# Bob-cheng/DepthModelHardening

Measured on AMD Instinct MI355X. Metric: adv-train images/sec @1024x320, 10-step PGD, bs32, higher is better.
Workload: dtype f32; 1 GPU; Monodepth2 ResNet18 1024x320, 10-step PGD-L_inf attack on 12 scenes, train batch 32/GPU, stereo photometric+SSIM+smoothness loss (md2), Adam; config_index=2, global_batch=32, per_gpu_batch=32, parallelism=dp1, attack_overlap=False, attack_scenes=12, graph_attack=False

## Files before the change

depthmodelhardening_amd/_native.py:

```python
import ctypes as C
import os

import torch

MAX_SCALES = 4
MAX_FRAMES = 4
VARIANT_MD2, VARIANT_DH = 0, 1
NOISE_NONE, NOISE_TENSOR, NOISE_PHILOX = 0, 1, 2
PASTE_COMPOSITE, PASTE_WARP_ONLY = 0, 1
FIN_LOSS, FIN_LOSS_S, FIN_REPROJ_S, FIN_COUNT_S, FIN_SMOOTH_S, FIN_HINT_S, FIN_HINTCOUNT_S, FIN_SIZE = 0, 1, 5, 9, 13, 20, 24, 28

LIB_PATH = os.environ.get("DMH_HIP_LIB") or os.path.join(os.path.dirname(os.path.abspath(__file__)), "lib",
                                                        "libdmh_hip.so")

_fp = C.c_void_p


class PhotoArgs(C.Structure):
    _fields_ = [("target", _fp), ("source", _fp * MAX_FRAMES), ("T", _fp * MAX_FRAMES), ("K", _fp), ("inv_K", _fp),
                ("disp", _fp * MAX_SCALES), ("Hs", C.c_int * MAX_SCALES), ("Ws", C.c_int * MAX_SCALES),
                ("B", C.c_int), ("H", C.c_int), ("W", C.c_int), ("num_frames", C.c_int), ("num_scales", C.c_int),
                ("min_depth", C.c_float), ("max_depth", C.c_float), ("variant", C.c_int), ("automask", C.c_int),
                ("no_ssim", C.c_int), ("noise_mode", C.c_int), ("noise", _fp * MAX_SCALES),
                ("seed", C.c_uint64), ("offset", C.c_uint64), ("depth_hint", _fp), ("depth_hint_mask", _fp)]
# ... 91 lines not shown
    "dmh_conv7x7s2_bwd_data_win": (C.c_int, [_fp] * 4 + [C.c_int] * 9 + [_fp, _fp]),
    "dmh_roi_cost_partials_size": (C.c_int64, [C.c_int, C.c_int, C.c_int]),
    "dmh_roi_cost_fwd": (C.c_int, [_fp, _fp, _fp] + [C.c_int] * 5 + [_fp] * 4),
    "dmh_roi_cost_bwd": (C.c_int, [_fp, _fp, _fp] + [C.c_int] * 5 + [_fp] * 3),
    "dmh_roi_cost_fwd_scaled": (C.c_int, [_fp, _fp, _fp] + [C.c_int] * 5 + [C.c_float] + [_fp] * 4),
    "dmh_roi_cost_bwd_scaled": (C.c_int, [_fp, _fp, _fp] + [C.c_int] * 5 + [C.c_float] + [_fp] * 3),
    "dmh_bn_act_fwd": (C.c_int, [_fp] * 4 + [C.c_int] * 4 + [_fp, _fp]),
    "dmh_bn_act_bwd": (C.c_int, [_fp] * 3 + [C.c_int] * 4 + [_fp, _fp, _fp]),
    "dmh_bn_stats_partials_size": (C.c_int64, [C.c_int, C.c_int, C.c_int]),
    "dmh_bn_train_stats": (C.c_int, [_fp, C.c_int, C.c_int, C.c_int, _fp, _fp, C.c_float, C.c_float] + [_fp] * 8),
    "dmh_bn_train_stats_tracked": (C.c_int, [_fp, C.c_int, C.c_int, C.c_int, _fp, _fp, C.c_float, C.c_float] + [_fp] * 9),
    "dmh_channel_sum_partials_size": (C.c_int64, [C.c_int, C.c_int, C.c_int]),
    "dmh_channel_sum": (C.c_int, [_fp, C.c_int, C.c_int, C.c_int, _fp, _fp, C.c_void_p]),
    "dmh_bn_train_bwd_workspace_size": (C.c_int64, [C.c_int, C.c_int, C.c_int]),
    "dmh_bn_train_bwd": (C.c_int, [_fp] * 6 + [C.c_int, C.c_int, C.c_int] + [_fp] * 5 + [C.c_void_p]),
    "dmh_stem_bn_relu_pool_fwd": (C.c_int, [_fp] * 3 + [C.c_int] * 4 + [_fp] * 4),
    "dmh_stem_bn_relu_pool_bwd": (C.c_int, [_fp] * 5 + [C.c_int] * 4 + [_fp, _fp]),
    "dmh_wino_weight_size": (C.c_int64, [C.c_int, C.c_int]),
    "dmh_wino_weight_transform": (C.c_int, [_fp, C.c_int, C.c_int, C.c_int, _fp, _fp]),
    "dmh_wino_conv3x3": (C.c_int, [_fp] * 3 + [C.c_int] * 6 + [_fp, _fp]),
    "dmh_wino_conv3x3_ws": (C.c_int, [_fp] * 3 + [C.c_int] * 6 + [_fp, _fp, C.c_int64, _fp]),
    "dmh_wino_conv3x3_plan": (C.c_int, [C.c_int] * 7 + [C.c_int64]),
    "dmh_wino_weight_transform_scaled": (C.c_int, [_fp, C.c_int, C.c_int, C.c_int, _fp, _fp, _fp]),
    "dmh_wino_conv3x3_act": (C.c_int, [_fp] * 4 + [C.c_int] * 7 + [_fp, _fp]),
    "dmh_wino_weight_transform_batch": (C.c_int, [C.POINTER(WinoWtJob), C.c_int, _fp]),
    "dmh_wino_conv3x3_act_ws": (C.c_int, [_fp] * 4 + [C.c_int] * 7 + [_fp, _fp, C.c_int64, _fp]),
    "dmh_wino32_weight_size": (C.c_int64, [C.c_int, C.c_int]),
    "dmh_wino32_weight_transform": (C.c_int, [_fp, C.c_int, C.c_int, C.c_int, _fp, _fp]),
    "dmh_wino32_conv3x3": (C.c_int, [_fp] * 3 + [C.c_int] * 6 + [_fp, _fp]),
    "dmh_wino32_conv3x3_ws": (C.c_int, [_fp] * 3 + [C.c_int] * 6 + [_fp, _fp, C.c_int64, _fp]),
# ... 88 lines not shown
```

depthmodelhardening_amd/csrc/encoder_glue.hip:

```cpp
#include "common.hpp"

#include <cmath>

using namespace dmh;

namespace {

constexpr int NT = 256;

__device__ __forceinline__ float relu_f(float v) { return v > 0.f ? v : 0.f; }

template <bool RELU, bool RES>
__global__ __launch_bounds__(NT) void bn_act_fwd_vec(const float4* __restrict__ x, const float* __restrict__ scale,
                                                     const float* __restrict__ shift, const float4* __restrict__ res,
                                                     unsigned C, unsigned hw4, unsigned total4, float4* __restrict__ out) {
    const unsigned i = blockIdx.x * NT + threadIdx.x;
    if (i >= total4) return;
    const unsigned c = (i / hw4) % C;
    const float s = scale[c], b = shift[c];
    const float4 v = x[i];
    float4 r = make_float4(fmaf(v.x, s, b), fmaf(v.y, s, b), fmaf(v.z, s, b), fmaf(v.w, s, b));
    if (RES) {
        const float4 q = res[i];
        r.x += q.x; r.y += q.y; r.z += q.z; r.w += q.w;
// ... 31 lines not shown
}

template <bool RELU, bool RES>
__global__ __launch_bounds__(NT) void bn_act_bwd_scalar(const float* __restrict__ out, const float* __restrict__ g,
                                                        const float* __restrict__ scale, unsigned C, unsigned hw,
                                                        unsigned total, float* __restrict__ g_x, float* __restrict__ g_res) {
    const unsigned i = blockIdx.x * NT + threadIdx.x;
    if (i >= total) return;
    float gv = g[i];
    if (RELU) gv = out[i] > 0.f ? gv : 0.f;
    if (RES) g_res[i] = gv;
    g_x[i] = gv * scale[(i / hw) % C];
}

__global__ __launch_bounds__(NT) void stem_fwd_kernel(const float* __restrict__ x, const float* __restrict__ scale,
                                                      const float* __restrict__ shift, int C, int H, int W,
                                                      float* __restrict__ feat, float* __restrict__ pooled,
                                                      unsigned char* __restrict__ argmax) {
    const int PH = H >> 1, PW = W >> 1;
    const int t = blockIdx.x * NT + threadIdx.x;
    if (t >= PH * PW) return;
    const int plane = blockIdx.y, c = plane % C;
    const int i = t / PW, j = t - i * PW;
    const float s = scale[c], b = shift[c];
    const float* xp = x + (size_t)plane * H * W;
    float* fp = feat + (size_t)plane * H * W;
    float m = -INFINITY;
    int arg = 4;
#pragma unroll
    for (int ky = 0; ky < 3; ++ky) {
        const int yy = 2 * i - 1 + ky;
        if (yy < 0) continue;
        const float* row = xp + (size_t)yy * W + 2 * j;
        const float2 vc = *reinterpret_cast<const float2*>(row);
        const float a1 = relu_f(fmaf(vc.x, s, b)), a2 = relu_f(fmaf(vc.y, s, b));
        if (j > 0) {
            const float a0 = relu_f(fmaf(row[-1], s, b));
// ... 112 lines not shown
    const int nslab = (HW + 4 * NT - 1) / (4 * NT);
    return s < nslab ? (nslab - 1 - s) / S + 1 : 0;
}

struct Wf {
    float n, mean, m2;
};
__device__ __forceinline__ Wf wf_merge(Wf a, Wf b) {
    if (b.n == 0.f) return a;
    if (a.n == 0.f) return b;
    const float n = a.n + b.n, d = b.mean - a.mean, f = b.n / n;
    return Wf{n, a.mean + d * f, a.m2 + b.m2 + d * d * a.n * f};
}

__global__ __launch_bounds__(NT) void bn_stats_partial_kernel(const float* __restrict__ x, int B, int C, int HW, int S,
                                                              float* __restrict__ part) {
    const int c = blockIdx.y, s = blockIdx.x;
    const float k = x[(size_t)c * HW];
    float nq[4] = {0.f, 0.f, 0.f, 0.f}, s1q[4] = {0.f, 0.f, 0.f, 0.f}, s2q[4] = {0.f, 0.f, 0.f, 0.f};
    for (int b = 0; b < B; ++b) {
        const float* xp = x + ((size_t)b * C + c) * HW;
        if ((HW & 3) == 0) continue;
        for (int r0 = s * 4 * NT; r0 < HW; r0 += S * 4 * NT) {
            float v[4];
#pragma unroll
            for (int q = 0; q < 4; ++q) {
                const int r = r0 + q * NT + threadIdx.x;
                v[q] = r < HW ? xp[r] : k;
                nq[q] += r < HW ? 1.f : 0.f;
            }
#pragma unroll
            for (int q = 0; q < 4; ++q) {
// ... 35 lines not shown
        Wf other{__shfl_down(w.n, o, WAVE), __shfl_down(w.mean, o, WAVE), __shfl_down(w.m2, o, WAVE)};
        w = wf_merge(w, other);
    }
    __shared__ Wf red[NT / WAVE];
    if ((threadIdx.x & (WAVE - 1)) == 0) red[threadIdx.x / WAVE] = w;
    __syncthreads();
    if (threadIdx.x == 0) {
        Wf t = red[0];
#pragma unroll
        for (int i = 1; i < NT / WAVE; ++i) t = wf_merge(t, red[i]);
        float* p = part + ((size_t)c * S + s) * 3;
        p[0] = t.n; p[1] = t.mean; p[2] = t.m2;
    }
}

__global__ __launch_bounds__(NT) void bn_stats_finalize_kernel(const float* __restrict__ part, int C, int S,
                                                               const float* __restrict__ weight,
                                                               const float* __restrict__ bias, float momentum, float eps,
                                                               float* __restrict__ running_mean,
                                                               float* __restrict__ running_var, float* __restrict__ scale,
                                                               float* __restrict__ shift, float* __restrict__ save_mean,
                                                               float* __restrict__ save_invstd,
                                                               long long* __restrict__ num_batches_tracked) {
    const int c = blockIdx.x * NT + threadIdx.x;
    if (c >= C) return;
    if (c == 0 && num_batches_tracked) num_batches_tracked[0] += 1;
    Wf t{0.f, 0.f, 0.f};
    for (int s = 0; s < S; ++s) {
        const float* p = part + ((size_t)c * S + s) * 3;
        t = wf_merge(t, Wf{p[0], p[1], p[2]});
    }
    const float var = t.m2 / t.n, invstd = rsqrtf(var + eps);
    const float sc = (weight ? weight[c] : 1.f) * invstd;
    scale[c] = sc;
    shift[c] = (bias ? bias[c] : 0.f) - t.mean * sc;
    save_mean[c] = t.mean;
    save_invstd[c] = invstd;
    if (running_mean) running_mean[c] = (1.f - momentum) * running_mean[c] + momentum * t.mean;
    if (running_var) running_var[c] = (1.f - momentum) * running_var[c] + momentum * (t.m2 / fmaxf(t.n - 1.f, 1.f));
}

inline unsigned blocks_for(int64_t n) { return (unsigned)((n + NT - 1) / NT); }

template <bool RELU, bool VEC>
__global__ __launch_bounds__(NT) void bn_bwd_partial_kernel(const float* __restrict__ x, const float* __restrict__ g,
                                                            const float* __restrict__ out, const float* __restrict__ mean,
                                                            int B, int C, int HW, int S, float* __restrict__ part) {
    const int c = blockIdx.y, s = blockIdx.x;
    const float m = mean[c];
    float a1[4] = {0.f, 0.f, 0.f, 0.f}, a2[4] = {0.f, 0.f, 0.f, 0.f};
    for (int b = 0; b < B; ++b) {
        const size_t base = ((size_t)b * C + c) * HW;
        if (VEC) {
            break;
        } else {
            for (int r0 = s * 4 * NT; r0 < HW; r0 += S * 4 * NT) {
#pragma unroll
                for (int q = 0; q < 4; ++q) {
                    const int r = r0 + q * NT + (int)threadIdx.x;
                    if (r < HW) {
                        float gv = g[base + r];
                        if (RELU) gv = out[base + r] > 0.f ? gv : 0.f;
                        a1[q] += gv;
// ... 40 lines not shown
        red[threadIdx.x / WAVE][1] = s2;
    }
    __syncthreads();
    if (threadIdx.x == 0) {
        float t1 = red[0][0], t2 = red[0][1];
#pragma unroll
        for (int i = 1; i < NT / WAVE; ++i) {
            t1 += red[i][0];
            t2 += red[i][1];
        }
        part[((size_t)c * S + s) * 2 + 0] = t1;
        part[((size_t)c * S + s) * 2 + 1] = t2;
    }
}

__global__ __launch_bounds__(NT) void bn_bwd_finalize_kernel(const float* __restrict__ part, int C, int S, double inv_n,
                                                             const float* __restrict__ weight, const float* __restrict__ mean,
                                                             const float* __restrict__ invstd, float* __restrict__ coef,
                                                             float* __restrict__ g_weight, float* __restrict__ g_bias) {
    const int c = blockIdx.x * NT + threadIdx.x;
    if (c >= C) return;
    double s1 = 0.0, s2 = 0.0;
    for (int s = 0; s < S; ++s) {
        s1 += (double)part[((size_t)c * S + s) * 2 + 0];
        s2 += (double)part[((size_t)c * S + s) * 2 + 1];
    }
    const double is = (double)invstd[c], w = weight ? (double)weight[c] : 1.0;
    if (g_bias) g_bias[c] = (float)s1;
    if (g_weight) g_weight[c] = (float)(s2 * is);
    float4 k;
    k.x = (float)(w * is);
    k.y = (float)(s1 * inv_n);
    k.z = (float)(s2 * is * is * inv_n);
    k.w = mean[c];
    reinterpret_cast<float4*>(coef)[c] = k;
}

template <bool RELU, bool RES>
__global__ __launch_bounds__(NT) void bn_bwd_apply_vec(const float4* __restrict__ x, const float4* __restrict__ g,
                                                       const float4* __restrict__ out, const float4* __restrict__ coef,
                                                       unsigned C, unsigned hw4, unsigned total4, float4* __restrict__ g_x,
                                                       float4* __restrict__ g_res) {
    const unsigned i = blockIdx.x * NT + threadIdx.x;
    if (i >= total4) return;
    const float4 k = coef[(i / hw4) % C];
    const float4 xv = x[i];
    float4 gv = g[i];
    if (RELU) {
        const float4 o = out[i];
        gv = make_float4(o.x > 0.f ? gv.x : 0.f, o.y > 0.f ? gv.y : 0.f, o.z > 0.f ? gv.z : 0.f, o.w > 0.f ? gv.w : 0.f);
    }
    if (RES) g_res[i] = gv;
    g_x[i] = make_float4(k.x * ((gv.x - k.y) - (xv.x - k.w) * k.z), k.x * ((gv.y - k.y) - (xv.y - k.w) * k.z),
                         k.x * ((gv.z - k.y) - (xv.z - k.w) * k.z), k.x * ((gv.w - k.y) - (xv.w - k.w) * k.z));
}

template <bool RELU, bool RES>
__global__ __launch_bounds__(NT) void bn_bwd_apply_scalar(const float* __restrict__ x, const float* __restrict__ g,
                                                          const float* __restrict__ out, const float4* __restrict__ coef,
                                                          unsigned C, unsigned hw, unsigned total, float* __restrict__ g_x,
                                                          float* __restrict__ g_res) {
    const unsigned i = blockIdx.x * NT + threadIdx.x;
    if (i >= total) return;
    const float4 k = coef[(i / hw) % C];
    float gv = g[i];
    if (RELU) gv = out[i] > 0.f ? gv : 0.f;
    if (RES) g_res[i] = gv;
    g_x[i] = k.x * ((gv - k.y) - (x[i] - k.w) * k.z);
}

template <bool RELU, bool RES>
void launch_bn_bwd_apply(const float* x, const float* g, const float* out, const float* coef, int C, int HW, int64_t total,
                         float* g_x, float* g_res, hipStream_t st) {
    if ((HW & 3) == 0)
        hipLaunchKernelGGL((bn_bwd_apply_vec<RELU, RES>), dim3(blocks_for(total / 4)), dim3(NT), 0, st,
                           reinterpret_cast<const float4*>(x), reinterpret_cast<const float4*>(g),
                           reinterpret_cast<const float4*>(out), reinterpret_cast<const float4*>(coef), (unsigned)C,
                           (unsigned)(HW / 4), (unsigned)(total / 4), reinterpret_cast<float4*>(g_x),
                           reinterpret_cast<float4*>(g_res));
    else
        hipLaunchKernelGGL((bn_bwd_apply_scalar<RELU, RES>), dim3(blocks_for(total)), dim3(NT), 0, st, x, g, out,
                           reinterpret_cast<const float4*>(coef), (unsigned)C, (unsigned)HW, (unsigned)total, g_x, g_res);
}

__global__ __launch_bounds__(NT) void channel_sum_partial_kernel(const float* __restrict__ g, int B, int C, int HW, int S,
                                                                 float* __restrict__ part) {
    const int c = blockIdx.y, s = blockIdx.x;
    float a[4] = {0.f, 0.f, 0.f, 0.f};
    if ((HW & 3) == 0) {
        const int nk = slabs_of(HW, s, S), total = B * nk;
        for (int i0 = 0; i0 < total; i0 += 4) {
            float4 v[4];
#pragma unroll
            for (int u = 0; u < 4; ++u) {
                const int i = min(i0 + u, total - 1), b = i / nk, r = (s + (i - b * nk) * S) * 4 * NT + 4 * (int)threadIdx.x;
                v[u] = (i0 + u < total && r < HW) ? *reinterpret_cast<const float4*>(g + ((size_t)b * C + c) * HW + r)
                                                  : make_float4(0.f, 0.f, 0.f, 0.f);
// ... 105 lines not shown
                       float* save_mean, float* save_invstd, void* stream) {
    return dmh_bn_train_stats_tracked(x, B, C, HW, weight, bias, momentum, eps, running_mean, running_var, nullptr, partials,
                                      scale, shift, save_mean, save_invstd, stream);
}

int dmh_bn_train_stats_tracked(const float* x, int B, int C, int HW, const float* weight, const float* bias, float momentum,
                               float eps, float* running_mean, float* running_var, long long* num_batches_tracked,
                               float* partials, float* scale, float* shift, float* save_mean, float* save_invstd,
                               void* stream) {
    DMH_REQUIRE(x && partials && scale && shift && save_mean && save_invstd, "null pointer");
    DMH_REQUIRE((reinterpret_cast<uintptr_t>(num_batches_tracked) & 7) == 0, "num_batches_tracked must be an aligned int64");
    DMH_REQUIRE(B > 0 && C > 0 && HW > 0 && C <= 65535, "bad sizes");
    int64_t S = ((int64_t)HW + 4 * NT - 1) / (4 * NT);
    if (S > 64) S = 64;
    hipStream_t st = (hipStream_t)stream;
    hipLaunchKernelGGL(bn_stats_partial_kernel, dim3((unsigned)S, C), dim3(NT), 0, st, x, B, C, HW, (int)S, partials);
    hipLaunchKernelGGL(bn_stats_finalize_kernel, dim3(blocks_for(C)), dim3(NT), 0, st, partials, C, (int)S, weight, bias,
                       momentum, eps, running_mean, running_var, scale, shift, save_mean, save_invstd, num_batches_tracked);
    return check_launch("dmh_bn_train_stats");
}

int64_t dmh_channel_sum_partials_size(int B, int C, int HW) {
    const int64_t S = dmh_bn_stats_partials_size(B, C, HW);
    return S < 0 ? -1 : S / 3;
}

int dmh_channel_sum(const float* g, int B, int C, int HW, float* partials, float* out, void* stream) {
    DMH_REQUIRE(g && partials && out, "null pointer");
    DMH_REQUIRE(B > 0 && C > 0 && HW > 0 && C <= 65535, "bad sizes");
    int64_t S = ((int64_t)HW + 4 * NT - 1) / (4 * NT);
    if (S > 64) S = 64;
    hipStream_t st = (hipStream_t)stream;
    hipLaunchKernelGGL(channel_sum_partial_kernel, dim3((unsigned)S, C), dim3(NT), 0, st, g, B, C, HW, (int)S, partials);
    hipLaunchKernelGGL(channel_sum_finalize_kernel, dim3(blocks_for(C)), dim3(NT), 0, st, partials, C, (int)S, out);
// ... 7 lines not shown
}

int dmh_bn_train_bwd(const float* x, const float* g_out, const float* out, const float* weight, const float* save_mean,
                     const float* save_invstd, int B, int C, int HW, float* workspace, float* g_x, float* g_weight,
                     float* g_bias, float* g_pre, void* stream) {
    DMH_REQUIRE(x && g_out && save_mean && save_invstd && workspace && g_x, "null pointer");
    DMH_REQUIRE(B > 0 && C > 0 && HW > 0 && C <= 65535, "bad sizes");
    const int64_t total = (int64_t)B * C * HW;
    DMH_REQUIRE(total < ((int64_t)1 << 31), "tensor too large");
    DMH_REQUIRE((reinterpret_cast<uintptr_t>(workspace) & 15) == 0, "workspace must be 16-byte aligned");
    int64_t S = ((int64_t)HW + 4 * NT - 1) / (4 * NT);
    if (S > 64) S = 64;
    hipStream_t st = (hipStream_t)stream;
    float* coef = workspace;
    float* part = workspace + (size_t)C * 4;
    const dim3 pg((unsigned)S, C);
    const bool vec = (HW & 3) == 0;
    if (out) {
        if (vec) hipLaunchKernelGGL((bn_bwd_partial_kernel<true, true>), pg, dim3(NT), 0, st, x, g_out, out, save_mean, B, C, HW, (int)S, part);
        else hipLaunchKernelGGL((bn_bwd_partial_kernel<true, false>), pg, dim3(NT), 0, st, x, g_out, out, save_mean, B, C, HW, (int)S, part);
    } else {
        if (vec) hipLaunchKernelGGL((bn_bwd_partial_kernel<false, true>), pg, dim3(NT), 0, st, x, g_out, out, save_mean, B, C, HW, (int)S, part);
        else hipLaunchKernelGGL((bn_bwd_partial_kernel<false, false>), pg, dim3(NT), 0, st, x, g_out, out, save_mean, B, C, HW, (int)S, part);
    }
    hipLaunchKernelGGL(bn_bwd_finalize_kernel, dim3(blocks_for(C)), dim3(NT), 0, st, part, C, (int)S,
                       1.0 / ((double)B * (double)HW), weight, save_mean, save_invstd, coef, g_weight, g_bias);
    if (out) {
        if (g_pre) launch_bn_bwd_apply<true, true>(x, g_out, out, coef, C, HW, total, g_x, g_pre, st);
        else launch_bn_bwd_apply<true, false>(x, g_out, out, coef, C, HW, total, g_x, nullptr, st);
    } else {
        if (g_pre) launch_bn_bwd_apply<false, true>(x, g_out, out, coef, C, HW, total, g_x, g_pre, st);
        else launch_bn_bwd_apply<false, false>(x, g_out, out, coef, C, HW, total, g_x, nullptr, st);
    }
    return check_launch("dmh_bn_train_bwd");
}

int dmh_stem_bn_relu_pool_fwd(const float* x, const float* scale, const float* shift, int B, int C, int H, int W,
                              float* feat, float* pooled, unsigned char* argmax, void* stream) {
    DMH_REQUIRE(x && scale && shift && feat && pooled && argmax, "null pointer");
    DMH_REQUIRE(B > 0 && C > 0 && H >= 2 && W >= 2 && (H & 1) == 0 && (W & 1) == 0, "H and W must be even and >= 2");
    DMH_REQUIRE((int64_t)B * C <= 65535 && (int64_t)H * W < (1 << 30), "tensor too large");
    hipLaunchKernelGGL(stem_fwd_kernel, dim3(blocks_for((int64_t)(H / 2) * (W / 2)), B * C), dim3(NT), 0,
                       (hipStream_t)stream, x, scale, shift, C, H, W, feat, pooled, argmax);
    return check_launch("dmh_stem_bn_relu_pool_fwd");
}

int dmh_stem_bn_relu_pool_bwd(const float* feat, const unsigned char* argmax, const float* g_feat, const float* g_pooled,
                              const float* scale, int B, int C, int H, int W, float* g_x, void* stream) {
    DMH_REQUIRE(feat && argmax && scale && g_x, "null pointer");
    DMH_REQUIRE(B > 0 && C > 0 && H >= 2 && W >= 2 && (H & 1) == 0 && (W & 1) == 0, "H and W must be even and >= 2");
    DMH_REQUIRE((int64_t)B * C <= 65535 && (int64_t)H * W < (1 << 30), "tensor too large");
    if ((W & 3) == 0)
        hipLaunchKernelGGL(stem_bwd4_kernel, dim3(blocks_for((int64_t)(H / 2) * (W / 4)), B * C), dim3(NT), 0,
                           (hipStream_t)stream, feat, argmax, g_feat, g_pooled, scale, C, H, W, g_x);
    else
        hipLaunchKernelGGL(stem_bwd_kernel, dim3(blocks_for((int64_t)(H / 2) * (W / 2)), B * C), dim3(NT), 0,
                           (hipStream_t)stream, feat, argmax, g_feat, g_pooled, scale, C, H, W, g_x);
    return check_launch("dmh_stem_bn_relu_pool_bwd");
// ... 4 lines not shown
```

depthmodelhardening_amd/ops.py:

```python
import contextlib
import ctypes as C
import os
from collections import namedtuple

import numpy as np
import torch

from . import _native as N

LossOut = namedtuple("LossOut", ["fin", "sel", "to_opt"])

_profile = None
_profile_only = None


def enable_profile(on=True, only=None):
    global _profile, _profile_only
    _profile = {} if on else None
    _profile_only = tuple(only) if (on and only) else None


def profile_ms():
    if not _profile:
        return {}
# ... 877 lines not shown
        return g_x, None, None, g_res, None


def _reject_affine_grad(name, scale, shift):
    if torch.is_grad_enabled() and not _wino_frozen and (scale.requires_grad or shift.requires_grad):
        raise RuntimeError("%s: scale/shift require grad, but this op treats them as constants (eval-mode BatchNorm "
                           "inside an attack); use the nn.BatchNorm2d module path, ops.frozen_weights() or detach()" % name)


def bn_act(x, scale, shift, residual=None, relu=True):
    _reject_affine_grad("bn_act", scale, shift)
    return _BnAct.apply(_c(x), _c(scale.detach()), _c(shift.detach()), None if residual is None else _c(residual),
                        bool(relu))


def _bn_train_stats(x, bn):
    lib = N.lib()
    B, Cc = x.shape[0], x.shape[1]
    HW = x.numel() // (B * Cc)
    dev = x.device
    part = torch.empty(lib.dmh_bn_stats_partials_size(B, Cc, HW), device=dev, dtype=torch.float32)
    scale, shift, mean, invstd = (torch.empty(Cc, device=dev, dtype=torch.float32) for _ in range(4))
    if bn.momentum is None:
        raise RuntimeError("bn_act_train: cumulative-average BatchNorm (momentum=None) is not supported")
    track = bn.track_running_stats and bn.running_mean is not None
    nbt = bn.num_batches_tracked if (track and bn.num_batches_tracked is not None) else None
    if nbt is not None and not (nbt.is_cuda and nbt.dtype == torch.int64 and nbt.numel() == 1):
        raise RuntimeError("bn_act_train: num_batches_tracked must be a CUDA int64 scalar")
    N.check(_timed("bn_train_stats", lambda: lib.dmh_bn_train_stats_tracked(
        N.ptr(x), B, Cc, HW, N.ptr(None if bn.weight is None else _c(bn.weight.detach())),
        N.ptr(None if bn.bias is None else _c(bn.bias.detach())), float(bn.momentum), float(bn.eps),
        N.ptr(bn.running_mean if track else None), N.ptr(bn.running_var if track else None),
        None if nbt is None else C.c_void_p(nbt.data_ptr()), N.ptr(part), N.ptr(scale),
        N.ptr(shift), N.ptr(mean), N.ptr(invstd), N.stream()), 4 * x.numel()))
    return scale, shift, mean, invstd


def _bn_backward(g_pre, x, weight, bn, mean, invstd, eps, mask):
    if all(mask) and weight is not None and hasattr(torch.ops.aten, "miopen_batch_norm_backward"):
        return torch.ops.aten.miopen_batch_norm_backward(x, g_pre, weight, bn.running_mean, bn.running_var, mean, invstd, eps)
    return torch.ops.aten.native_batch_norm_backward(g_pre, x, weight, bn.running_mean, bn.running_var, mean, invstd, True,
                                                     eps, mask)


def channel_sum(g):
    lib = N.lib()
    B, Cc = g.shape[0], g.shape[1]
    HW = g.numel() // (B * Cc)
    part = torch.empty(lib.dmh_channel_sum_partials_size(B, Cc, HW), device=g.device, dtype=torch.float32)
    out = torch.empty(Cc, device=g.device, dtype=torch.float32)
# ... 14 lines not shown
    gw = torch.empty(Cc, device=g.device, dtype=torch.float32)
    gb = torch.empty(Cc, device=g.device, dtype=torch.float32)
    g_pre = torch.empty_like(g) if want_pre else None
    nb = 4 * g.numel() * ((6 if out is not None else 4) + 1 + (1 if want_pre else 0))
    N.check(_timed("bn_train_bwd", lambda: lib.dmh_bn_train_bwd(
        N.ptr(x), N.ptr(g), N.ptr(out), N.ptr(weight), N.ptr(mean), N.ptr(invstd), B, Cc, HW, N.ptr(ws), N.ptr(gx), N.ptr(gw),
        N.ptr(gb), N.ptr(g_pre), N.stream()), nb))
    return gx, gw, gb, g_pre


class _BnActTrain(torch.autograd.Function):

    @staticmethod
    def forward(ctx, x, weight, bias, residual, relu, bn):
        lib = N.lib()
        scale, shift, mean, invstd = _bn_train_stats(x, bn)
        B, Cc = x.shape[0], x.shape[1]
        HW = x.numel() // (B * Cc)
        out = torch.empty_like(x)
        nb = 4 * (x.numel() * (2 if residual is None else 3))
        N.check(_timed("bn_act_fwd", lambda: lib.dmh_bn_act_fwd(N.ptr(x), N.ptr(scale), N.ptr(shift), N.ptr(residual), B, Cc,
                                                               HW, int(relu), N.ptr(out), N.stream()), nb))
        ctx.save_for_backward(x, weight, mean, invstd, out if relu else None)
        ctx.relu, ctx.eps, ctx.bn = bool(relu), float(bn.eps), bn
        ctx.res_grad = residual is not None and residual.requires_grad
        return out

    @staticmethod
    def backward(ctx, g):
        x, weight, mean, invstd, out = ctx.saved_tensors
        lib = N.lib()
        g = _c(g)
        B, Cc = g.shape[0], g.shape[1]
        if BN_BWD_ENABLED and weight is not None and g.numel() < (1 << 31) and Cc <= 65535:
            gx, gw, gb, g_pre = _bn_backward_fused(g, x, out if ctx.relu else None, weight, mean, invstd,
                                                   ctx.res_grad and ctx.relu)
            if ctx.res_grad and not ctx.relu:
# ... 45 lines not shown
        g_pooled = None if g_pooled is None else _c(g_pooled)
        g_x = torch.empty_like(feat)
        nb = 4 * (2 * feat.numel() + (0 if g_feat is None else feat.numel()) +
                  (0 if g_pooled is None else g_pooled.numel())) + arg.numel()
        N.check(_timed("stem_bwd", lambda: lib.dmh_stem_bn_relu_pool_bwd(N.ptr(feat), N.ptr(arg), N.ptr(g_feat),
                                                                        N.ptr(g_pooled), N.ptr(scale), B, Cc, H, W,
                                                                        N.ptr(g_x), N.stream()), nb))
        return g_x, None, None


class _StemTrain(torch.autograd.Function):

    @staticmethod
    def forward(ctx, x, weight, bias, bn):
        lib = N.lib()
        scale, shift, mean, invstd = _bn_train_stats(x, bn)
        B, Cc, H, W = x.shape
        feat = torch.empty_like(x)
        pooled = torch.empty((B, Cc, H // 2, W // 2), device=x.device, dtype=torch.float32)
        arg = torch.empty((B, Cc, H // 2, W // 2), device=x.device, dtype=torch.uint8)
        nb = 4 * (2 * x.numel() + pooled.numel()) + arg.numel()
        N.check(_timed("stem_fwd", lambda: lib.dmh_stem_bn_relu_pool_fwd(N.ptr(x), N.ptr(scale), N.ptr(shift), B, Cc, H, W,
                                                                        N.ptr(feat), N.ptr(pooled), N.ptr(arg),
                                                                        N.stream()), nb))
        ctx.save_for_backward(x, weight, mean, invstd, feat, arg)
        ctx.eps, ctx.bn = float(bn.eps), bn
        ctx.mark_non_differentiable(arg)
        ctx.set_materialize_grads(False)
        return feat, pooled, arg

    @staticmethod
    def backward(ctx, g_feat, g_pooled, _g_arg):
        x, weight, mean, invstd, feat, arg = ctx.saved_tensors
        if g_feat is None and g_pooled is None:
            return None, None, None, None
        lib = N.lib()
        B, Cc, H, W = feat.shape
        g_feat = None if g_feat is None else _c(g_feat)
        g_pooled = None if g_pooled is None else _c(g_pooled)
# ... 1473 lines not shown
```

include/dmh_hip.h:

```cpp
#ifndef DMH_HIP_H
#define DMH_HIP_H

#include <stdint.h>

#ifdef __cplusplus
extern "C" {
#endif

#define DMH_OK 0
#define DMH_EINVAL 1
#define DMH_ELAUNCH 2

#define DMH_MAX_SCALES 4
#define DMH_MAX_FRAMES 4

#define DMH_VARIANT_MD2 0
#define DMH_VARIANT_DH 1

#define DMH_NOISE_NONE 0
#define DMH_NOISE_TENSOR 1
#define DMH_NOISE_PHILOX 2

#define DMH_FIN_LOSS 0
#define DMH_FIN_LOSS_S 1
// ... 226 lines not shown
                   float* g_residual, void* stream);
int64_t dmh_bn_stats_partials_size(int B, int C, int HW);
int dmh_bn_train_stats(const float* x, int B, int C, int HW, const float* weight, const float* bias, float momentum,
                       float eps, float* running_mean, float* running_var, float* partials, float* scale, float* shift,
                       float* save_mean, float* save_invstd, void* stream);
int dmh_bn_train_stats_tracked(const float* x, int B, int C, int HW, const float* weight, const float* bias, float momentum,
                               float eps, float* running_mean, float* running_var, long long* num_batches_tracked,
                               float* partials, float* scale, float* shift, float* save_mean, float* save_invstd,
                               void* stream);
int64_t dmh_channel_sum_partials_size(int B, int C, int HW);
int dmh_channel_sum(const float* g, int B, int C, int HW, float* partials, float* out, void* stream);
int64_t dmh_bn_train_bwd_workspace_size(int B, int C, int HW);
int dmh_bn_train_bwd(const float* x, const float* g_out, const float* out, const float* weight, const float* save_mean,
                     const float* save_invstd, int B, int C, int HW, float* workspace, float* g_x, float* g_weight,
                     float* g_bias, float* g_pre, void* stream);
int dmh_stem_bn_relu_pool_fwd(const float* x, const float* scale, const float* shift, int B, int C, int H, int W,
                              float* feat, float* pooled, unsigned char* argmax, void* stream);
int dmh_stem_bn_relu_pool_bwd(const float* feat, const unsigned char* argmax, const float* g_feat, const float* g_pooled,
                              const float* scale, int B, int C, int H, int W, float* g_x, void* stream);

int64_t dmh_wino_weight_size(int n_out, int n_in);
int dmh_wino_weight_transform(const float* w, int K, int C, int backward, float* U, void* stream);
int dmh_wino_conv3x3(const float* x, const float* U, const float* bias, int B, int C, int K, int H, int W, int pad,
                     float* y, void* stream);
int dmh_wino_conv3x3_ws(const float* x, const float* U, const float* bias, int B, int C, int K, int H, int W, int pad,
                        float* y, float* workspace, int64_t workspace_floats, void* stream);
int dmh_wino_conv3x3_plan(int B, int C, int K, int H, int W, int pad, int epilogue, int64_t workspace_floats);
int dmh_wino_weight_transform_scaled(const float* w, int K, int C, int backward, const float* scale, float* U,
                                     void* stream);
int dmh_wino_conv3x3_act(const float* x, const float* U, const float* bias, const float* residual, int relu, int B, int C,
// ... 67 lines not shown
```

Measured before the change: 407.7 images/s.

## Add channel-grouped BatchNorm train forward/backward to keep slices cache-resident

Adds combined BN-train forward entry points (stats, finalize, apply) for regular and stem layers. They can split channels into groups sized to an env-controlled memory budget, so the apply pass re-reads data that is still in cache, optionally visiting blocks in reverse order. The budget defaults to zero, so by default there is a single group and the main effect is merging the stats and apply calls into one native call, which removes some Python/ctypes overhead. It also adds index arithmetic inside the apply kernels.

```diff
diff --git a/depthmodelhardening_amd/_native.py b/depthmodelhardening_amd/_native.py
--- a/depthmodelhardening_amd/_native.py
+++ b/depthmodelhardening_amd/_native.py
@@ -129,6 +129,10 @@
     "dmh_channel_sum": (C.c_int, [_fp, C.c_int, C.c_int, C.c_int, _fp, _fp, C.c_void_p]),
     "dmh_bn_train_bwd_workspace_size": (C.c_int64, [C.c_int, C.c_int, C.c_int]),
     "dmh_bn_train_bwd": (C.c_int, [_fp] * 6 + [C.c_int, C.c_int, C.c_int] + [_fp] * 5 + [C.c_void_p]),
+    "dmh_bn_group_width": (C.c_int, [C.c_int] * 4),
+    "dmh_bn_train_fwd": (C.c_int, [_fp, C.c_int, C.c_int, C.c_int, _fp, _fp, C.c_float, C.c_float] + [_fp] * 5 + [C.c_int]
+                         + [_fp] * 6),
+    "dmh_stem_bn_train_fwd": (C.c_int, [_fp] + [C.c_int] * 4 + [_fp, _fp, C.c_float, C.c_float] + [_fp] * 12),
     "dmh_stem_bn_relu_pool_fwd": (C.c_int, [_fp] * 3 + [C.c_int] * 4 + [_fp] * 4),
     "dmh_stem_bn_relu_pool_bwd": (C.c_int, [_fp] * 5 + [C.c_int] * 4 + [_fp, _fp]),
     "dmh_wino_weight_size": (C.c_int64, [C.c_int, C.c_int]),
diff --git a/depthmodelhardening_amd/csrc/encoder_glue.hip b/depthmodelhardening_amd/csrc/encoder_glue.hip
--- a/depthmodelhardening_amd/csrc/encoder_glue.hip
+++ b/depthmodelhardening_amd/csrc/encoder_glue.hip
@@ -1,6 +1,7 @@
 #include "common.hpp"
 
 #include <cmath>
+#include <cstdlib>
 
 using namespace dmh;
 
@@ -69,13 +70,13 @@
 }
 
 __global__ __launch_bounds__(NT) void stem_fwd_kernel(const float* __restrict__ x, const float* __restrict__ scale,
-                                                      const float* __restrict__ shift, int C, int H, int W,
+                                                      const float* __restrict__ shift, int C, int c0, int G, int H, int W,
                                                       float* __restrict__ feat, float* __restrict__ pooled,
                                                       unsigned char* __restrict__ argmax) {
     const int PH = H >> 1, PW = W >> 1;
     const int t = blockIdx.x * NT + threadIdx.x;
     if (t >= PH * PW) return;
-    const int plane = blockIdx.y, c = plane % C;
+    const int bi = blockIdx.y / G, c = c0 + blockIdx.y - bi * G, plane = bi * C + c;
     const int i = t / PW, j = t - i * PW;
     const float s = scale[c], b = shift[c];
     const float* xp = x + (size_t)plane * H * W;
@@ -218,8 +219,8 @@
 }
 
 __global__ __launch_bounds__(NT) void bn_stats_partial_kernel(const float* __restrict__ x, int B, int C, int HW, int S,
-                                                              float* __restrict__ part) {
-    const int c = blockIdx.y, s = blockIdx.x;
+                                                              int c0, float* __restrict__ part) {
+    const int c = c0 + blockIdx.y, s = blockIdx.x;
     const float k = x[(size_t)c * HW];
     float nq[4] = {0.f, 0.f, 0.f, 0.f}, s1q[4] = {0.f, 0.f, 0.f, 0.f}, s2q[4] = {0.f, 0.f, 0.f, 0.f};
     for (int b = 0; b < B; ++b) {
@@ -285,7 +286,7 @@
     }
 }
 
-__global__ __launch_bounds__(NT) void bn_stats_finalize_kernel(const float* __restrict__ part, int C, int S,
+__global__ __launch_bounds__(NT) void bn_stats_finalize_kernel(const float* __restrict__ part, int c0, int G, int S,
                                                                const float* __restrict__ weight,
                                                                const float* __restrict__ bias, float momentum, float eps,
                                                                float* __restrict__ running_mean,
@@ -293,8 +294,8 @@
                                                                float* __restrict__ shift, float* __restrict__ save_mean,
                                                                float* __restrict__ save_invstd,
                                                                long long* __restrict__ num_batches_tracked) {
-    const int c = blockIdx.x * NT + threadIdx.x;
-    if (c >= C) return;
+    const int cg = blockIdx.x * NT + threadIdx.x, c = c0 + cg;
+    if (cg >= G) return;
     if (c == 0 && num_batches_tracked) num_batches_tracked[0] += 1;
     Wf t{0.f, 0.f, 0.f};
     for (int s = 0; s < S; ++s) {
@@ -316,8 +317,8 @@
 template <bool RELU, bool VEC>
 __global__ __launch_bounds__(NT) void bn_bwd_partial_kernel(const float* __restrict__ x, const float* __restrict__ g,
                                                             const float* __restrict__ out, const float* __restrict__ mean,
-                                                            int B, int C, int HW, int S, float* __restrict__ part) {
-    const int c = blockIdx.y, s = blockIdx.x;
+                                                            int B, int C, int HW, int S, int c0, float* __restrict__ part) {
+    const int c = c0 + blockIdx.y, s = blockIdx.x;
     const float m = mean[c];
     float a1[4] = {0.f, 0.f, 0.f, 0.f}, a2[4] = {0.f, 0.f, 0.f, 0.f};
     for (int b = 0; b < B; ++b) {
@@ -388,12 +389,12 @@
     }
 }
 
-__global__ __launch_bounds__(NT) void bn_bwd_finalize_kernel(const float* __restrict__ part, int C, int S, double inv_n,
+__global__ __launch_bounds__(NT) void bn_bwd_finalize_kernel(const float* __restrict__ part, int c0, int G, int S, double inv_n,
                                                              const float* __restrict__ weight, const float* __restrict__ mean,
                                                              const float* __restrict__ invstd, float* __restrict__ coef,
                                                              float* __restrict__ g_weight, float* __restrict__ g_bias) {
-    const int c = blockIdx.x * NT + threadIdx.x;
-    if (c >= C) return;
+    const int cg = blockIdx.x * NT + threadIdx.x, c = c0 + cg;
+    if (cg >= G) return;
     double s1 = 0.0, s2 = 0.0;
     for (int s = 0; s < S; ++s) {
         s1 += (double)part[((size_t)c * S + s) * 2 + 0];
@@ -410,14 +411,39 @@
     reinterpret_cast<float4*>(coef)[c] = k;
 }
 
+struct Grp {
+    unsigned B, C, hw, c0, G, rev;
+};
+__device__ __forceinline__ bool grp_index(const Grp& q, unsigned total, unsigned& i, unsigned& c) {
+    const unsigned j = (q.rev ? gridDim.x - 1 - blockIdx.x : blockIdx.x) * NT + threadIdx.x;
+    if (j >= total) return false;
+    unsigned b, cg, r;
+    if (q.rev) {
+        const unsigned bhw = q.B * q.hw;
+        cg = j / bhw;
+        const unsigned rem = j - cg * bhw;
+        b = rem / q.hw;
+        r = rem - b * q.hw;
+    } else {
+        const unsigned ghw = q.G * q.hw;
+        b = j / ghw;
+        const unsigned rem = j - b * ghw;
+        cg = rem / q.hw;
+        r = rem - cg * q.hw;
+    }
+    c = q.c0 + cg;
+    i = (b * q.C + c) * q.hw + r;
+    return true;
+}
+
 template <bool RELU, bool RES>
 __global__ __launch_bounds__(NT) void bn_bwd_apply_vec(const float4* __restrict__ x, const float4* __restrict__ g,
                                                        const float4* __restrict__ out, const float4* __restrict__ coef,
-                                                       unsigned C, unsigned hw4, unsigned total4, float4* __restrict__ g_x,
+                                                       Grp q, unsigned total4, float4* __restrict__ g_x,
                                                        float4* __restrict__ g_res) {
-    const unsigned i = blockIdx.x * NT + threadIdx.x;
-    if (i >= total4) return;
-    const float4 k = coef[(i / hw4) % C];
+    unsigned i, c;
+    if (!grp_index(q, total4, i, c)) return;
+    const float4 k = coef[c];
     const float4 xv = x[i];
     float4 gv = g[i];
     if (RELU) {
@@ -432,29 +458,91 @@
 template <bool RELU, bool RES>
 __global__ __launch_bounds__(NT) void bn_bwd_apply_scalar(const float* __restrict__ x, const float* __restrict__ g,
                                                           const float* __restrict__ out, const float4* __restrict__ coef,
-                                                          unsigned C, unsigned hw, unsigned total, float* __restrict__ g_x,
+                                                          Grp q, unsigned total, float* __restrict__ g_x,
                                                           float* __restrict__ g_res) {
-    const unsigned i = blockIdx.x * NT + threadIdx.x;
-    if (i >= total) return;
-    const float4 k = coef[(i / hw) % C];
+    unsigned i, c;
+    if (!grp_index(q, total, i, c)) return;
+    const float4 k = coef[c];
     float gv = g[i];
     if (RELU) gv = out[i] > 0.f ? gv : 0.f;
     if (RES) g_res[i] = gv;
     g_x[i] = k.x * ((gv - k.y) - (x[i] - k.w) * k.z);
 }
 
-template <bool RELU, bool RES>
-void launch_bn_bwd_apply(const float* x, const float* g, const float* out, const float* coef, int C, int HW, int64_t total,
+inline Grp grp_of(int B, int C, int HW, int c0, int G, bool rev) {
+    return Grp{(unsigned)B, (unsigned)C, (unsigned)((HW & 3) == 0 ? HW / 4 : HW), (unsigned)c0, (unsigned)G, rev ? 1u : 0u};
+}
+
+template <bool RELU, bool RES>
+void launch_bn_bwd_apply(const float* x, const float* g, const float* out, const float* coef, int HW, const Grp& q,
                          float* g_x, float* g_res, hipStream_t st) {
+    const unsigned total = q.B * q.G * q.hw;
     if ((HW & 3) == 0)
-        hipLaunchKernelGGL((bn_bwd_apply_vec<RELU, RES>), dim3(blocks_for(total / 4)), dim3(NT), 0, st,
+        hipLaunchKernelGGL((bn_bwd_apply_vec<RELU, RES>), dim3(blocks_for(total)), dim3(NT), 0, st,
                            reinterpret_cast<const float4*>(x), reinterpret_cast<const float4*>(g),
-                           reinterpret_cast<const float4*>(out), reinterpret_cast<const float4*>(coef), (unsigned)C,
-                           (unsigned)(HW / 4), (unsigned)(total / 4), reinterpret_cast<float4*>(g_x),
-                           reinterpret_cast<float4*>(g_res));
+                           reinterpret_cast<const float4*>(out), reinterpret_cast<const float4*>(coef), q, total,
+                           reinterpret_cast<float4*>(g_x), reinterpret_cast<float4*>(g_res));
     else
         hipLaunchKernelGGL((bn_bwd_apply_scalar<RELU, RES>), dim3(blocks_for(total)), dim3(NT), 0, st, x, g, out,
-                           reinterpret_cast<const float4*>(coef), (unsigned)C, (unsigned)HW, (unsigned)total, g_x, g_res);
+                           reinterpret_cast<const float4*>(coef), q, total, g_x, g_res);
+}
+
+template <bool RELU, bool RES>
+__global__ __launch_bounds__(NT) void bn_train_act_vec(const float4* __restrict__ x, const float* __restrict__ scale,
+                                                       const float* __restrict__ shift, const float4* __restrict__ res, Grp q,
+                                                       unsigned total4, float4* __restrict__ out) {
+    unsigned i, c;
+    if (!grp_index(q, total4, i, c)) return;
+    const float s = scale[c], b = shift[c];
+    const float4 v = x[i];
+    float4 r = make_float4(fmaf(v.x, s, b), fmaf(v.y, s, b), fmaf(v.z, s, b), fmaf(v.w, s, b));
+    if (RES) {
+        const float4 w = res[i];
+        r.x += w.x; r.y += w.y; r.z += w.z; r.w += w.w;
+    }
+    if (RELU) r = make_float4(relu_f(r.x), relu_f(r.y), relu_f(r.z), relu_f(r.w));
+    out[i] = r;
+}
+
+template <bool RELU, bool RES>
+__global__ __launch_bounds__(NT) void bn_train_act_scalar(const float* __restrict__ x, const float* __restrict__ scale,
+                                                          const float* __restrict__ shift, const float* __restrict__ res, Grp q,
+                                                          unsigned total, float* __restrict__ out) {
+    unsigned i, c;
+    if (!grp_index(q, total, i, c)) return;
+    float r = fmaf(x[i], scale[c], shift[c]);
+    if (RES) r += res[i];
+    out[i] = RELU ? relu_f(r) : r;
+}
+
+template <bool RELU, bool RES>
+void launch_bn_train_act(const float* x, const float* scale, const float* shift, const float* res, int HW, const Grp& q,
+                         float* out, hipStream_t st) {
+    const unsigned total = q.B * q.G * q.hw;
+    if ((HW & 3) == 0)
+        hipLaunchKernelGGL((bn_train_act_vec<RELU, RES>), dim3(blocks_for(total)), dim3(NT), 0, st,
+                           reinterpret_cast<const float4*>(x), scale, shift, reinterpret_cast<const float4*>(res), q, total,
+                           reinterpret_cast<float4*>(out));
+    else
+        hipLaunchKernelGGL((bn_train_act_scalar<RELU, RES>), dim3(blocks_for(total)), dim3(NT), 0, st, x, scale, shift, res, q,
+                           total, out);
+}
+
+constexpr double BN_GROUP_MB_DEFAULT = 0.0;
+inline double bn_group_mb() {
+    const char* e = std::getenv("DMH_BN_GROUP_MB");
+    const double v = e && *e ? std::atof(e) : BN_GROUP_MB_DEFAULT;
+    return v > 0.0 ? v : 0.0;
+}
+inline int bn_group_width(int n_tensors, int B, int C, int HW) {
+    const double budget = bn_group_mb() * 1048576.0, per_channel = (double)n_tensors * B * HW * 4.0;
+    if (budget <= 0.0 || per_channel * C <= budget) return C;
+    const double g = std::floor(budget / per_channel);
+    return g < 1.0 ? 1 : (int)g;
+}
+inline bool bn_group_rev() {
+    const char* e = std::getenv("DMH_BN_GROUP_REV");
+    return e && *e ? std::atoi(e) != 0 : true;
 }
 
 __global__ __launch_bounds__(NT) void channel_sum_partial_kernel(const float* __restrict__ g, int B, int C, int HW, int S,
@@ -590,10 +678,71 @@
     int64_t S = ((int64_t)HW + 4 * NT - 1) / (4 * NT);
     if (S > 64) S = 64;
     hipStream_t st = (hipStream_t)stream;
-    hipLaunchKernelGGL(bn_stats_partial_kernel, dim3((unsigned)S, C), dim3(NT), 0, st, x, B, C, HW, (int)S, partials);
-    hipLaunchKernelGGL(bn_stats_finalize_kernel, dim3(blocks_for(C)), dim3(NT), 0, st, partials, C, (int)S, weight, bias,
+    hipLaunchKernelGGL(bn_stats_partial_kernel, dim3((unsigned)S, C), dim3(NT), 0, st, x, B, C, HW, (int)S, 0, partials);
+    hipLaunchKernelGGL(bn_stats_finalize_kernel, dim3(blocks_for(C)), dim3(NT), 0, st, partials, 0, C, (int)S, weight, bias,
                        momentum, eps, running_mean, running_var, scale, shift, save_mean, save_invstd, num_batches_tracked);
     return check_launch("dmh_bn_train_stats");
+}
+
+int dmh_bn_group_width(int n_tensors, int B, int C, int HW) {
+    if (n_tensors <= 0 || B <= 0 || C <= 0 || HW <= 0) return -1;
+    return bn_group_width(n_tensors, B, C, HW);
+}
+
+int dmh_bn_train_fwd(const float* x, int B, int C, int HW, const float* weight, const float* bias, float momentum, float eps,
+                     float* running_mean, float* running_var, long long* num_batches_tracked, float* partials,
+                     const float* residual, int relu, float* scale, float* shift, float* save_mean, float* save_invstd,
+                     float* out, void* stream) {
+    DMH_REQUIRE(x && partials && scale && shift && save_mean && save_invstd && out, "null pointer");
+    DMH_REQUIRE((reinterpret_cast<uintptr_t>(num_batches_tracked) & 7) == 0, "num_batches_tracked must be an aligned int64");
+    DMH_REQUIRE(B > 0 && C > 0 && HW > 0 && C <= 65535, "bad sizes");
+    DMH_REQUIRE((int64_t)B * C * HW < ((int64_t)1 << 31), "tensor too large");
+    int64_t S = ((int64_t)HW + 4 * NT - 1) / (4 * NT);
+    if (S > 64) S = 64;
+    hipStream_t st = (hipStream_t)stream;
+    const int GW = bn_group_width(residual ? 2 : 1, B, C, HW);
+    const bool rev = GW < C && bn_group_rev();
+    for (int c0 = 0; c0 < C; c0 += GW) {
+        const int G = C - c0 < GW ? C - c0 : GW;
+        hipLaunchKernelGGL(bn_stats_partial_kernel, dim3((unsigned)S, G), dim3(NT), 0, st, x, B, C, HW, (int)S, c0, partials);
+        hipLaunchKernelGGL(bn_stats_finalize_kernel, dim3(blocks_for(G)), dim3(NT), 0, st, partials, c0, G, (int)S, weight,
+                           bias, momentum, eps, running_mean, running_var, scale, shift, save_mean, save_invstd,
+                           num_batches_tracked);
+        const Grp q = grp_of(B, C, HW, c0, G, rev);
+        if (relu) {
+            if (residual) launch_bn_train_act<true, true>(x, scale, shift, residual, HW, q, out, st);
+            else launch_bn_train_act<true, false>(x, scale, shift, nullptr, HW, q, out, st);
+        } else {
+            if (residual) launch_bn_train_act<false, true>(x, scale, shift, residual, HW, q, out, st);
+            else launch_bn_train_act<false, false>(x, scale, shift, nullptr, HW, q, out, st);
+        }
+    }
+    return check_launch("dmh_bn_train_fwd");
+}
+
+int dmh_stem_bn_train_fwd(const float* x, int B, int C, int H, int W, const float* weight, const float* bias, float momentum,
+                          float eps, float* running_mean, float* running_var, long long* num_batches_tracked, float* partials,
+                          float* scale, float* shift, float* save_mean, float* save_invstd, float* feat, float* pooled,
+                          unsigned char* argmax, void* stream) {
+    DMH_REQUIRE(x && partials && scale && shift && save_mean && save_invstd && feat && pooled && argmax, "null pointer");
+    DMH_REQUIRE((reinterpret_cast<uintptr_t>(num_batches_tracked) & 7) == 0, "num_batches_tracked must be an aligned int64");
+    DMH_REQUIRE(B > 0 && C > 0 && H >= 2 && W >= 2 && (H & 1) == 0 && (W & 1) == 0, "H and W must be even and >= 2");
+    DMH_REQUIRE((int64_t)B * C <= 65535 && (int64_t)H * W < (1 << 30), "tensor too large");
+    const int HW = H * W;
+    int64_t S = ((int64_t)HW + 4 * NT - 1) / (4 * NT);
+    if (S > 64) S = 64;
+    hipStream_t st = (hipStream_t)stream;
+    const int GW = bn_group_width(1, B, C, HW);
+    for (int c0 = 0; c0 < C; c0 += GW) {
+        const int G = C - c0 < GW ? C - c0 : GW;
+        hipLaunchKernelGGL(bn_stats_partial_kernel, dim3((unsigned)S, G), dim3(NT), 0, st, x, B, C, HW, (int)S, c0, partials);
+        hipLaunchKernelGGL(bn_stats_finalize_kernel, dim3(blocks_for(G)), dim3(NT), 0, st, partials, c0, G, (int)S, weight,
+                           bias, momentum, eps, running_mean, running_var, scale, shift, save_mean, save_invstd,
+                           num_batches_tracked);
+        hipLaunchKernelGGL(stem_fwd_kernel, dim3(blocks_for((int64_t)(H / 2) * (W / 2)), B * G), dim3(NT), 0, st, x, scale,
+                           shift, C, c0, G, H, W, feat, pooled, argmax);
+    }
+    return check_launch("dmh_stem_bn_train_fwd");
 }
 
 int64_t dmh_channel_sum_partials_size(int B, int C, int HW) {
@@ -631,23 +780,29 @@
     hipStream_t st = (hipStream_t)stream;
     float* coef = workspace;
     float* part = workspace + (size_t)C * 4;
-    const dim3 pg((unsigned)S, C);
     const bool vec = (HW & 3) == 0;
-    if (out) {
-        if (vec) hipLaunchKernelGGL((bn_bwd_partial_kernel<true, true>), pg, dim3(NT), 0, st, x, g_out, out, save_mean, B, C, HW, (int)S, part);
-        else hipLaunchKernelGGL((bn_bwd_partial_kernel<true, false>), pg, dim3(NT), 0, st, x, g_out, out, save_mean, B, C, HW, (int)S, part);
-    } else {
-        if (vec) hipLaunchKernelGGL((bn_bwd_partial_kernel<false, true>), pg, dim3(NT), 0, st, x, g_out, out, save_mean, B, C, HW, (int)S, part);
-        else hipLaunchKernelGGL((bn_bwd_partial_kernel<false, false>), pg, dim3(NT), 0, st, x, g_out, out, save_mean, B, C, HW, (int)S, part);
-    }
-    hipLaunchKernelGGL(bn_bwd_finalize_kernel, dim3(blocks_for(C)), dim3(NT), 0, st, part, C, (int)S,
-                       1.0 / ((double)B * (double)HW), weight, save_mean, save_invstd, coef, g_weight, g_bias);
-    if (out) {
-        if (g_pre) launch_bn_bwd_apply<true, true>(x, g_out, out, coef, C, HW, total, g_x, g_pre, st);
-        else launch_bn_bwd_apply<true, false>(x, g_out, out, coef, C, HW, total, g_x, nullptr, st);
-    } else {
-        if (g_pre) launch_bn_bwd_apply<false, true>(x, g_out, out, coef, C, HW, total, g_x, g_pre, st);
-        else launch_bn_bwd_apply<false, false>(x, g_out, out, coef, C, HW, total, g_x, nullptr, st);
+    const int GW = bn_group_width(out ? 3 : 2, B, C, HW);
+    const bool rev = GW < C && bn_group_rev();
+    for (int c0 = 0; c0 < C; c0 += GW) {
+        const int G = C - c0 < GW ? C - c0 : GW;
+        const dim3 pg((unsigned)S, G);
+        if (out) {
+            if (vec) hipLaunchKernelGGL((bn_bwd_partial_kernel<true, true>), pg, dim3(NT), 0, st, x, g_out, out, save_mean, B, C, HW, (int)S, c0, part);
+            else hipLaunchKernelGGL((bn_bwd_partial_kernel<true, false>), pg, dim3(NT), 0, st, x, g_out, out, save_mean, B, C, HW, (int)S, c0, part);
+        } else {
+            if (vec) hipLaunchKernelGGL((bn_bwd_partial_kernel<false, true>), pg, dim3(NT), 0, st, x, g_out, out, save_mean, B, C, HW, (int)S, c0, part);
+            else hipLaunchKernelGGL((bn_bwd_partial_kernel<false, false>), pg, dim3(NT), 0, st, x, g_out, out, save_mean, B, C, HW, (int)S, c0, part);
+        }
+        hipLaunchKernelGGL(bn_bwd_finalize_kernel, dim3(blocks_for(G)), dim3(NT), 0, st, part, c0, G, (int)S,
+                           1.0 / ((double)B * (double)HW), weight, save_mean, save_invstd, coef, g_weight, g_bias);
+        const Grp q = grp_of(B, C, HW, c0, G, rev);
+        if (out) {
+            if (g_pre) launch_bn_bwd_apply<true, true>(x, g_out, out, coef, HW, q, g_x, g_pre, st);
+            else launch_bn_bwd_apply<true, false>(x, g_out, out, coef, HW, q, g_x, nullptr, st);
+        } else {
+            if (g_pre) launch_bn_bwd_apply<false, true>(x, g_out, out, coef, HW, q, g_x, g_pre, st);
+            else launch_bn_bwd_apply<false, false>(x, g_out, out, coef, HW, q, g_x, nullptr, st);
+        }
     }
     return check_launch("dmh_bn_train_bwd");
 }
@@ -658,7 +813,7 @@
     DMH_REQUIRE(B > 0 && C > 0 && H >= 2 && W >= 2 && (H & 1) == 0 && (W & 1) == 0, "H and W must be even and >= 2");
     DMH_REQUIRE((int64_t)B * C <= 65535 && (int64_t)H * W < (1 << 30), "tensor too large");
     hipLaunchKernelGGL(stem_fwd_kernel, dim3(blocks_for((int64_t)(H / 2) * (W / 2)), B * C), dim3(NT), 0,
-                       (hipStream_t)stream, x, scale, shift, C, H, W, feat, pooled, argmax);
+                       (hipStream_t)stream, x, scale, shift, C, 0, C, H, W, feat, pooled, argmax);
     return check_launch("dmh_stem_bn_relu_pool_fwd");
 }
 
diff --git a/depthmodelhardening_amd/ops.py b/depthmodelhardening_amd/ops.py
--- a/depthmodelhardening_amd/ops.py
+++ b/depthmodelhardening_amd/ops.py
@@ -915,26 +915,32 @@
                         bool(relu))
 
 
-def _bn_train_stats(x, bn):
+def _bn_train_args(x, bn):
     lib = N.lib()
     B, Cc = x.shape[0], x.shape[1]
     HW = x.numel() // (B * Cc)
     dev = x.device
     part = torch.empty(lib.dmh_bn_stats_partials_size(B, Cc, HW), device=dev, dtype=torch.float32)
-    scale, shift, mean, invstd = (torch.empty(Cc, device=dev, dtype=torch.float32) for _ in range(4))
+    outs = tuple(torch.empty(Cc, device=dev, dtype=torch.float32) for _ in range(4))
     if bn.momentum is None:
         raise RuntimeError("bn_act_train: cumulative-average BatchNorm (momentum=None) is not supported")
     track = bn.track_running_stats and bn.running_mean is not None
     nbt = bn.num_batches_tracked if (track and bn.num_batches_tracked is not None) else None
     if nbt is not None and not (nbt.is_cuda and nbt.dtype == torch.int64 and nbt.numel() == 1):
         raise RuntimeError("bn_act_train: num_batches_tracked must be a CUDA int64 scalar")
+    keep = (None if bn.weight is None else _c(bn.weight.detach()), None if bn.bias is None else _c(bn.bias.detach()), part)
+    stats = (N.ptr(keep[0]), N.ptr(keep[1]), float(bn.momentum), float(bn.eps), N.ptr(bn.running_mean if track else None),
+             N.ptr(bn.running_var if track else None), None if nbt is None else C.c_void_p(nbt.data_ptr()), N.ptr(part))
+    return stats, outs, keep
+
+
+def _bn_train_stats(x, bn):
+    lib = N.lib()
+    B, Cc = x.shape[0], x.shape[1]
+    stats, outs, _keep = _bn_train_args(x, bn)
     N.check(_timed("bn_train_stats", lambda: lib.dmh_bn_train_stats_tracked(
-        N.ptr(x), B, Cc, HW, N.ptr(None if bn.weight is None else _c(bn.weight.detach())),
-        N.ptr(None if bn.bias is None else _c(bn.bias.detach())), float(bn.momentum), float(bn.eps),
-        N.ptr(bn.running_mean if track else None), N.ptr(bn.running_var if track else None),
-        None if nbt is None else C.c_void_p(nbt.data_ptr()), N.ptr(part), N.ptr(scale),
-        N.ptr(shift), N.ptr(mean), N.ptr(invstd), N.stream()), 4 * x.numel()))
-    return scale, shift, mean, invstd
+        N.ptr(x), B, Cc, x.numel() // (B * Cc), *stats, *(N.ptr(t) for t in outs), N.stream()), 4 * x.numel()))
+    return outs
 
 
 def _bn_backward(g_pre, x, weight, bn, mean, invstd, eps, mask):
@@ -979,13 +985,14 @@
     @staticmethod
     def forward(ctx, x, weight, bias, residual, relu, bn):
         lib = N.lib()
-        scale, shift, mean, invstd = _bn_train_stats(x, bn)
         B, Cc = x.shape[0], x.shape[1]
         HW = x.numel() // (B * Cc)
         out = torch.empty_like(x)
-        nb = 4 * (x.numel() * (2 if residual is None else 3))
-        N.check(_timed("bn_act_fwd", lambda: lib.dmh_bn_act_fwd(N.ptr(x), N.ptr(scale), N.ptr(shift), N.ptr(residual), B, Cc,
-                                                               HW, int(relu), N.ptr(out), N.stream()), nb))
+        stats, (scale, shift, mean, invstd), _keep = _bn_train_args(x, bn)
+        nb = 4 * (x.numel() * (3 if residual is None else 4))
+        N.check(_timed("bn_train_fwd", lambda: lib.dmh_bn_train_fwd(
+            N.ptr(x), B, Cc, HW, *stats, N.ptr(residual), int(relu), N.ptr(scale), N.ptr(shift), N.ptr(mean), N.ptr(invstd),
+            N.ptr(out), N.stream()), nb))
         ctx.save_for_backward(x, weight, mean, invstd, out if relu else None)
         ctx.relu, ctx.eps, ctx.bn = bool(relu), float(bn.eps), bn
         ctx.res_grad = residual is not None and residual.requires_grad
@@ -1061,15 +1068,17 @@
     @staticmethod
     def forward(ctx, x, weight, bias, bn):
         lib = N.lib()
-        scale, shift, mean, invstd = _bn_train_stats(x, bn)
         B, Cc, H, W = x.shape
+        if (H | W) & 1 or B * Cc > 65535 or H * W >= (1 << 30):
+            raise RuntimeError("stem_bn_relu_pool_train: H and W must be even, B * C <= 65535 (got %s)" % (tuple(x.shape),))
         feat = torch.empty_like(x)
         pooled = torch.empty((B, Cc, H // 2, W // 2), device=x.device, dtype=torch.float32)
         arg = torch.empty((B, Cc, H // 2, W // 2), device=x.device, dtype=torch.uint8)
-        nb = 4 * (2 * x.numel() + pooled.numel()) + arg.numel()
-        N.check(_timed("stem_fwd", lambda: lib.dmh_stem_bn_relu_pool_fwd(N.ptr(x), N.ptr(scale), N.ptr(shift), B, Cc, H, W,
-                                                                        N.ptr(feat), N.ptr(pooled), N.ptr(arg),
-                                                                        N.stream()), nb))
+        stats, (scale, shift, mean, invstd), _keep = _bn_train_args(x, bn)
+        nb = 4 * (3 * x.numel() + pooled.numel()) + arg.numel()
+        N.check(_timed("stem_train_fwd", lambda: lib.dmh_stem_bn_train_fwd(
+            N.ptr(x), B, Cc, H, W, *stats, N.ptr(scale), N.ptr(shift), N.ptr(mean), N.ptr(invstd), N.ptr(feat), N.ptr(pooled),
+            N.ptr(arg), N.stream()), nb))
         ctx.save_for_backward(x, weight, mean, invstd, feat, arg)
         ctx.eps, ctx.bn = float(bn.eps), bn
         ctx.mark_non_differentiable(arg)
diff --git a/include/dmh_hip.h b/include/dmh_hip.h
--- a/include/dmh_hip.h
+++ b/include/dmh_hip.h
@@ -264,6 +264,15 @@
 int dmh_bn_train_bwd(const float* x, const float* g_out, const float* out, const float* weight, const float* save_mean,
                      const float* save_invstd, int B, int C, int HW, float* workspace, float* g_x, float* g_weight,
                      float* g_bias, float* g_pre, void* stream);
+int dmh_bn_group_width(int n_tensors, int B, int C, int HW);
+int dmh_bn_train_fwd(const float* x, int B, int C, int HW, const float* weight, const float* bias, float momentum, float eps,
+                     float* running_mean, float* running_var, long long* num_batches_tracked, float* partials,
+                     const float* residual, int relu, float* scale, float* shift, float* save_mean, float* save_invstd,
+                     float* out, void* stream);
+int dmh_stem_bn_train_fwd(const float* x, int B, int C, int H, int W, const float* weight, const float* bias, float momentum,
+                          float eps, float* running_mean, float* running_var, long long* num_batches_tracked, float* partials,
+                          float* scale, float* shift, float* save_mean, float* save_invstd, float* feat, float* pooled,
+                          unsigned char* argmax, void* stream);
 int dmh_stem_bn_relu_pool_fwd(const float* x, const float* scale, const float* shift, int B, int C, int H, int W,
                               float* feat, float* pooled, unsigned char* argmax, void* stream);
 int dmh_stem_bn_relu_pool_bwd(const float* feat, const unsigned char* argmax, const float* g_feat, const float* g_pooled,
```

Measured after the change: 407.0 images/s. Within noise of the previous version (-0.2%).
